# big-nacho/patolette

Measured on AMD Instinct MI355X. Metric: Mpixels/sec quantized (256-color ICtCp + KMeans) at 1 GPU; palette ΔE vs ref, higher is better.
Workload: dtype f64

## Files before the change

patolette_amd/csrc/pipeline.hip:

```cpp
#include <algorithm>
#include <functional>
#include <chrono>
#include <cmath>
#include <atomic>
#include <memory>
#include <mutex>
#include <thread>
#include <future>

#include "color_device.h"
#include "common.h"
#include "host_math.h"
#include "kmeans.h"
#include "map.h"
#include "saliency.h"
#include "quant.h"
#include "rgba.h"
#include "compact.h"

namespace pamd {

void launch_convert(int which, const double *src, double *dst, size_t n, ConvertStats *stats, hipStream_t s, BinK sumk = BinK{0.0, 0.0},
                    BinK momk = BinK{0.0, 0.0}, size_t begin = 0, size_t end = ~(size_t)0, bool init_stats = true);
void launch_convert_rows(int which, const double *rows, double *dst, size_t n, ConvertStats *stats, hipStream_t s,
// ... 818 lines not shown
    PinBuf<ConvertStats> h_cstats;
    hipEvent_t ev_stats = nullptr;
    hipStream_t stream2 = nullptr;
    hipEvent_t ev_up[2] = {nullptr, nullptr}, ev_join = nullptr;
    size_t prep_N = 0, prep_planes = 0;
    DevBuf<double> src, wsrc, cvt, bufA, bufB, aux;
    DevBuf<unsigned short> bkt;
    DevBuf<NodeDev> nodes;
    DevBuf<NodeIn> stage_in;
    DevBuf<NodeOut> stage_out;
    DevBuf<int> ids, round_nodes, node_tile0;
    DevBuf<Tile> tilesA, tilesP;
    DevBuf<double> hist, sum6, dpal;
    DevBuf<unsigned long long> hsize, tileoff;
    DevBuf<unsigned int> hcount, tilecnt;
    DevBuf<unsigned char> lut, dmap, src8, pal8, quant8;
    DevBuf<unsigned> rgba_cnt;
    DevBuf<int> rgba_cpos;
    DevBuf<unsigned char> rgba_rgb, rgba_map;
    DevBuf<double> rgba_w;
    PinBuf<unsigned> h_rgba_m;
    DevBuf<ConvertStats> cstats;
    PinBuf<NodeIn> h_stage_in;
    PinBuf<NodeOut> h_stage_out;
    PinBuf<int> h_ids, h_ids_get;
    PinBuf<Tile> h_tilesA, h_tilesP;
    PinBuf<int> h_round, h_tile0;
    PinBuf<double> h_dbl;
    PinBuf<unsigned char> h_bytes, h_packet, h_mapstage;
    DevBuf<unsigned char> packet;
// ... 402 lines not shown

static bool lq_device_eligible(const Engine &E, size_t N, size_t K, bool verbose, bool allow_device) {
    const int lq_mode = g_lq_device.load(std::memory_order_relaxed);
    return allow_device && (lq_mode == 1 || (lq_mode == 2 && N < kLqDeviceAutoPixels)) && !E.shard && !verbose && K <= (size_t)kLqDevMaxK;
}

static void ws_prepare(Engine &E, size_t N, size_t K, bool weighted, bool verbose) {
    const size_t planes = weighted ? 4 : 3;
    const bool lq_dev = lq_device_eligible(E, N, K, verbose, true);
    const size_t slack = lq_dev ? (size_t)kLqRoundCap : 0, ntA = ceil_div(N, (size_t)kTileA) + slack, ntP = ceil_div(N, (size_t)kTileP) + slack;
    const size_t tables = lq_dev ? (size_t)kLqRoundCap * kBuckets : (size_t)kBuckets;
    E.cvt.reserve(planes * N); E.cstats.reserve(1);
    E.bufA.reserve(planes * N + 64); E.bufB.reserve(planes * N + 64); E.bkt.reserve(N);
    E.tilesA.reserve(ntA); E.tilesP.reserve(ntP);
    E.tilecnt.reserve(ntP * kMaxChildren); E.tileoff.reserve(ntP * kMaxChildren);
    E.round_nodes.reserve(1); E.node_tile0.reserve(2); E.h_round.reserve(kBuckets);
    E.hist.reserve(std::max(hist_slot_doubles(), lq_dev ? (size_t)kNQ_LQ * 2 * kBuckets * kLqRoundCap : 0));
    E.hsize.reserve(tables); E.hcount.reserve(tables); E.lut.reserve(tables);
    E.nodes.reserve(std::max<size_t>(4 * K + 64, lq_dev ? (size_t)kLqNodeCap : 0));
    E.h_dbl.reserve(16 * kBuckets * 2 + 64);
    E.gq.reserve(1); E.gqout.reserve(1); E.h_gqout.reserve(1); E.h_gq.reserve(1);
    const size_t nput = kGqMaxK + 1;
    E.stage_in.reserve(nput); E.stage_out.reserve(nput); E.ids.reserve(nput); E.h_stage_in.reserve(nput); E.h_stage_out.reserve(nput);
    E.h_ids.reserve(nput); E.h_ids_get.reserve(nput);
    E.h_cent.reserve(3 * K);
    if (lq_dev) { E.lqctl.reserve(1); E.h_lqhead.reserve(1); E.h_lqrec.reserve(kLqNodeCap); E.h_lqcen.reserve(kLqNodeCap); }
}

static int lq_device_loop(Engine &E, size_t N, size_t K, bool weighted, bool inv_sums, const Bounds &bnd, const QuantBuffers &qlq, int kbase,
                          int first_base, int nnodes, std::vector<double> &centers, size_t &len, unsigned long long *max_members) {
    hipStream_t s = E.stream;
    const size_t lqs = (size_t)kNQ_LQ * 2 * kBuckets;
    const int ntA_ub = (int)ceil_div(N, (size_t)kTileA) + kLqRoundCap, ntP_ub = (int)ceil_div(N, (size_t)kTileP) + kLqRoundCap;
    E.lqctl.reserve(1); E.h_lqhead.reserve(1); E.h_lqrec.reserve(kLqNodeCap); E.h_lqcen.reserve(kLqNodeCap);
    E.hist.reserve(std::max(hist_slot_doubles(), lqs * kLqRoundCap)); E.hsize.reserve((size_t)kLqRoundCap * kBuckets);
    E.hcount.reserve((size_t)kLqRoundCap * kBuckets); E.lut.reserve((size_t)kLqRoundCap * kBuckets);
    E.tilesA.reserve(ntA_ub); E.tilesP.reserve(ntP_ub);
    E.tilecnt.reserve((size_t)ntP_ub * kMaxChildren); E.tileoff.reserve((size_t)ntP_ub * kMaxChildren);
    LqCtl *c = E.lqctl.p;
    LqHead *head = E.h_lqhead.p;
    for (int r = 0; r < kLqMaxRounds; r++) { head->round_px[r] = 0.0; head->round_nr[r] = 0.0; }
    const RoundDyn *dyn = &c->dyn;
    const int *d_round = c->round_ids, *d_tP0 = c->tP0;
    int call = 0;
    const GqOut *gq = kbase < 0 ? (const GqOut *)E.gqout.p : nullptr;
    const int kb_ub = kbase < 0 ? kGqMaxK : kbase;
    auto control = [&]() {
        const bool first = call == 0;
        {
            KTIME("k_lq_children", s, 0.0);
            if (first) hipLaunchKernelGGL(k_lq_children, (kb_ub + 3) / 4, 256, 0, s, E.nodes.p, c, call, kb_ub, first_base, nnodes, (int)K, gq);
            else hipLaunchKernelGGL(k_lq_children, 2 * kLqRoundCap / 4, 256, 0, s, E.nodes.p, c, call, 0, 0, 0, 0, (const GqOut *)nullptr);
        }
        KTIME("k_lq_select", s, 0.0);
        hipLaunchKernelGGL(k_lq_select, 1 + (first ? (kb_ub + 3) / 4 : 2 * kLqRoundCap / 4), 256, 0, s, E.nodes.p, c, call, bnd.e_lin, bnd.e_quad);
        HIP_CHECK(hipGetLastError());
        call++;
    };
    int enq = 0;
    auto round = [&]() {
        if (enq >= kLqMaxRounds) throw HipError("patolette_amd: split loop exceeded its round limit");
        const double *px_src = &head->round_px[enq], *nr_src = &head->round_nr[enq];
        const bool rev = enq % 2 == 1;
        static const bool setup_kernel = getenv("PAMD_LQ_SETUP_KERNEL") && atoi(getenv("PAMD_LQ_SETUP_KERNEL")) != 0;
        if (setup_kernel) {
            hipLaunchKernelGGL(k_round_setup_dyn, 1024, 256, 0, s, E.nodes.p, (const LqCtl *)c, E.tilesA.p, E.tilesP.p, E.hist.p, E.hsize.p, E.hcount.p, lqs);
            HIP_CHECK(hipGetLastError());
            launch_minmax(qlq, E.tilesA.p, ntA_ub, 0, E.nodes.p, s, rev, dyn, px_src);
        } else {
            const RoundLists rl{c->round_ids, c->tA0, c->tP0, E.tilesA.p, E.tilesP.p, E.hist.p, lqs, E.hsize.p, E.hcount.p};
            launch_minmax(qlq, E.tilesA.p, ntA_ub, 0, E.nodes.p, s, rev, dyn, px_src, &rl);
        }
        launch_hist(qlq, false, E.tilesA.p, ntA_ub, 0, E.nodes.p, E.hist.p, E.hsize.p, E.hcount.p, s, !rev, false, dyn, px_src);
        launch_cut(weighted, E.nodes.p, d_round, kLqRoundCap, E.hist.p, E.hsize.p, E.hcount.p, E.lut.p, s, dyn, nr_src);
        launch_partition(qlq, E.tilesP.p, ntP_ub, 0, d_round, d_tP0, kLqRoundCap, E.nodes.p, E.lut.p, E.tilecnt.p, E.tileoff.p, true, s, inv_sums, rev, dyn, px_src);
        enq++;
        control();
    };
    control();
    int want = (E.lq_hint_N == N && E.lq_hint_K == K && E.lq_hint_rounds > 0) ? E.lq_hint_rounds : 9;
    const bool fault_full = g_debug_fault.load(std::memory_order_relaxed) == 4;
    if (fault_full) want = 3;
    for (;;) {
        while (enq < want) round();
        hipLaunchKernelGGL(k_lq_export, 16, 256, 0, s, (const LqCtl *)c, head, E.h_lqrec.p, E.h_lqcen.p);
        HIP_CHECK(hipGetLastError());
        E.sync();
        if (fault_full) return -2;
        if (head->done) break;
        want = enq + 2;
// ... 1918 lines not shown
```

patolette_amd/csrc/quant.h:

```cpp
#pragma once

#include <atomic>

#include "common.h"
#include "devutil.h"

namespace pamd {

constexpr int kMaxChildren = 16;
constexpr int kTileA = 8192;
constexpr int kTileP = 2048;

constexpr int kNQ_LQ = 4;
constexpr int kNQ_GQ = 14;

constexpr int kSlots = 16;

struct NodeIn {
    unsigned long long begin, n, gn;
    int buf, slot, child0, nchild;
    int split;
    double axis[3], mean[3], sw;
    BinK klin, kquad;
};
// ... 84 lines not shown
constexpr int kSum3Slots = 32;
void launch_sum3(const double *planar, size_t N, BinK k, double *d_out6, hipStream_t s);
constexpr int kGqMaxK = 12;
struct GqDpDev {
    unsigned long long w0[kBuckets + 1];
    double w1[3][kBuckets + 1], w2[kBuckets + 1];
    double E[2][kBuckets + 1];
    int cut[kGqMaxK + 1][kBuckets + 1];
};
void launch_gq_dp(const double *d_hist, const unsigned int *d_hcount, int kmax, GqDpDev *d_g, hipStream_t s);

void launch_minmax(const QuantBuffers &qb, const Tile *d_tiles, int ntiles, size_t px, NodeDev *d_nodes, hipStream_t s, bool from_end = false,
                   const RoundDyn *dyn = nullptr, const double *px_src = nullptr, const RoundLists *lists = nullptr);
void launch_hist(const QuantBuffers &qb, bool gq, const Tile *d_tiles, int ntiles, size_t px, NodeDev *d_nodes,
                 double *d_hist, unsigned long long *d_hsize, unsigned int *d_hcount, hipStream_t s, bool from_end = false,
                 bool fixed_point = false, const RoundDyn *dyn = nullptr, const double *px_src = nullptr);
void launch_cut(bool weighted, NodeDev *d_nodes, const int *d_round_nodes, int nround, const double *d_hist,
                const unsigned long long *d_hsize, const unsigned int *d_hcount, unsigned char *d_lut, hipStream_t s,
                const RoundDyn *dyn = nullptr, const double *nr_src = nullptr);
void launch_partition(const QuantBuffers &qb, const Tile *d_ptiles, int nptiles, size_t px, const int *d_round_nodes,
                      const int *d_node_tile0, int nround, NodeDev *d_nodes, const unsigned char *d_lut,
                      unsigned int *d_tilecnt, unsigned long long *d_tileoff, bool fuse_cov, hipStream_t s,
                      bool invariant = false, bool from_end = false, const RoundDyn *dyn = nullptr, const double *px_src = nullptr,
                      bool gated = false);
void launch_cov_children(const QuantBuffers &qb, const Tile *d_tiles, int ntiles, size_t px, NodeDev *d_nodes, hipStream_t s, bool from_end = false,
                         bool gated = false);
void launch_cov_nodes(const QuantBuffers &qb, const double *planar_override, const Tile *d_tiles, int ntiles, size_t px,
                      NodeDev *d_nodes, hipStream_t s, bool from_end = false);

extern std::atomic<int> g_debug_fault;
size_t hist_slot_doubles();

}
```

patolette_amd/csrc/quant.hip:

```cpp
#include "quant.h"

#include <atomic>

#include <type_traits>

namespace pamd {

template <typename T>
__device__ __forceinline__ T block_scan_incl(T v, T *smem) {
    const int lane = threadIdx.x & 63, wid = threadIdx.x >> 6, nw = blockDim.x >> 6;
#pragma unroll
    for (int o = 1; o < 64; o <<= 1) {
        T t = __shfl_up(v, o, 64);
        if (lane >= o) v += t;
    }
    __syncthreads();
    if (lane == 63) smem[wid] = v;
    __syncthreads();
    if (wid == 0) {
        T s = lane < nw ? smem[lane] : T(0);
#pragma unroll
        for (int o = 1; o < 16; o <<= 1) {
            T t = __shfl_up(s, o, 64);
            if (lane >= o) s += t;
// ... 107 lines not shown
#pragma unroll
    for (int o = 32; o > 0; o >>= 1) { mn = fmin(mn, __shfl_down(mn, o, 64)); mx = fmax(mx, __shfl_down(mx, o, 64)); }
    __shared__ double smn[4], smx[4];
    if ((threadIdx.x & 63) == 0) { smn[threadIdx.x >> 6] = mn; smx[threadIdx.x >> 6] = mx; }
    __syncthreads();
    if (threadIdx.x == 0) {
        for (int w = 1; w < 4; w++) { mn = fmin(mn, smn[w]); mx = fmax(mx, smx[w]); }
        if (mn <= mx) {
            atomicMin(&nd.minkey[blockIdx.x & (kSlots - 1)], f64_key(mn));
            atomicMax(&nd.maxkey[blockIdx.x & (kSlots - 1)], f64_key(mx));
        }
    }
}

constexpr int kHistCombineMin = 12;
template <bool W, bool GQ>
__global__ __launch_bounds__(512) void k_hist(QuantBuffers qb, const Tile *__restrict__ tiles, int ntiles, NodeDev *nodes,
                                              double *hist, unsigned long long *hsize, unsigned int *hcount, const int from_end,
                                              const RoundDyn *__restrict__ dyn) {
    constexpr int NQ = GQ ? (W ? 14 : 10) : (W ? 4 : 3);
    int nblk = (int)gridDim.x;
    if (dyn) {
        ntiles = dyn->ntA;
        nblk = min(ntiles, nblk);
        if ((int)blockIdx.x >= nblk) return;
    }
    constexpr int NQS = GQ ? kNQ_GQ : kNQ_LQ;
    extern __shared__ double lds[];
    double *h = lds;
    unsigned long long *siz = (unsigned long long *)(h + NQ * 2 * kBuckets);
    unsigned int *cnt = (unsigned int *)(siz + kBuckets);
    for (int i = threadIdx.x; i < NQ * 2 * kBuckets; i += blockDim.x) h[i] = 0.0;
    for (int i = threadIdx.x; i < kBuckets; i += blockDim.x) { cnt[i] = 0u; siz[i] = 0ULL; }
    __syncthreads();

    const int per = (ntiles + nblk - 1) / nblk;
    const int bid = from_end ? nblk - 1 - (int)blockIdx.x : (int)blockIdx.x;
    const int tfirst = bid * per, tlast = min(ntiles, tfirst + per);
    for (int ti = tfirst; ti < tlast; ti++) {
        const Tile t = tiles[ti];
        NodeDev &nd = nodes[t.node];
        const double a0 = nd.axis[0], a1 = nd.axis[1], a2 = nd.axis[2];
        double mn, mx;
        node_minmax(nd, mn, mx);
        const bool degenerate = (mx - mn < kDelta);
        const double sc = 1 / (mx - mn);
        const BinK klin = nd.klin, kquad = nd.kquad;
        const double *px = qb.buf[nd.buf], *py = px + qb.N, *pz = py + qb.N, *pw = pz + qb.N;
// ... 62 lines not shown
        for (; i + 512 < t.count; i += 1024) {
            const size_t p0 = t.start + i, p1 = p0 + 512;
            const double x0 = px[p0], y0 = py[p0], z0 = pz[p0], x1 = px[p1], y1 = py[p1], z1 = pz[p1];
            double w0 = 1.0, w1 = 1.0;
            if constexpr (W) { w0 = pw[p0]; w1 = pw[p1]; }
            one(p0, x0, y0, z0, w0);
            one(p1, x1, y1, z1, w1);
        }
        for (; i < t.count; i += 512) {
            const size_t p = t.start + i;
            double w = 1.0;
            if constexpr (W) w = pw[p];
            one(p, px[p], py[p], pz[p], w);
        }
        const bool flush = (ti + 1 == tlast) || tiles[ti + 1].node != t.node;
        if (!flush) continue;
        __syncthreads();
        const size_t slot = (size_t)nd.slot;
        double *gh = hist + slot * (size_t)(NQS * 2 * kBuckets);
        for (int i = threadIdx.x; i < NQ * 2 * kBuckets; i += blockDim.x) {
            double v = h[i];
            if (v != 0.0) { unsafeAtomicAdd(&gh[i], v); h[i] = 0.0; }
        }
        for (int b = threadIdx.x; b < kBuckets; b += blockDim.x) {
            unsigned c = cnt[b];
            if (c) { atomicAdd(&hcount[slot * kBuckets + b], c); cnt[b] = 0u; }
            if constexpr (W && !GQ) { const unsigned long long s = siz[b]; if (s) { atomicAdd(&hsize[slot * kBuckets + b], s); siz[b] = 0ULL; } }
        }
        __syncthreads();
    }
}

// ... 133 lines not shown
                h[i2] = 0ULL;
            }
        }
        for (int b = threadIdx.x; b < kBuckets; b += blockDim.x) {
            unsigned c = cnt[b];
            if (c) { atomicAdd(&hcount[slot * kBuckets + b], c); cnt[b] = 0u; }
            if constexpr (W && !GQ) { const unsigned long long s2 = siz[b]; if (s2) { atomicAdd(&hsize[slot * kBuckets + b], s2); siz[b] = 0ULL; } }
        }
        __syncthreads();
    }
}

template <bool W>
__global__ __launch_bounds__(512) void k_cut(NodeDev *nodes, const int *__restrict__ round_nodes, const double *__restrict__ hist,
                                             const unsigned long long *__restrict__ hsize, const unsigned int *__restrict__ hcount,
                                             unsigned char *lut, const int fault, const RoundDyn *__restrict__ dyn) {
    if (dyn && (int)blockIdx.x >= dyn->nr) return;
    __shared__ double sd[4 * 16];
    __shared__ unsigned long long su[2 * 16];
    __shared__ double best_v[8];
    __shared__ int best_i[8];
    __shared__ double tot[8];
    __shared__ unsigned long long tots[2];
    __shared__ int s_split;
    const int b = threadIdx.x;
    NodeDev &nd = nodes[round_nodes[blockIdx.x]];
    const size_t slot = (size_t)nd.slot;
    const double *gh = hist + slot * (size_t)(kNQ_LQ * 2 * kBuckets);
    constexpr int NQ = W ? 4 : 3;
    double p[NQ][2];
    {
// ... 67 lines not shown
            double s0[NQ], s1[NQ];
#pragma unroll
            for (int q = 0; q < NQ; q++) {
                s0[q] = side == 0 ? p[q][0] : tot[q * 2] - p[q][0];
                s1[q] = side == 0 ? p[q][1] : tot[q * 2 + 1] - p[q][1];
            }
            double sw = W ? (s0[NQ - 1] + s1[NQ - 1]) : (double)ch.n;
            ch.sw = sw;
            const double inv = 1 / sw;
            for (int j = 0; j < 3; j++) ch.mean[j] = (s0[j] + s1[j]) * inv;
            ch.axis[0] = ch.axis[1] = ch.axis[2] = 0;
        }
    }
    for (int i = b; i < 2 * kNodeResetElems; i += kBuckets)
        node_reset_element(nodes[nd.child0 + i / kNodeResetElems], i % kNodeResetElems);
}

__global__ __launch_bounds__(256) void k_count(QuantBuffers qb, const Tile *__restrict__ tiles, const NodeDev *__restrict__ nodes,
                                               const unsigned char *__restrict__ lut, unsigned int *tilecnt, const int from_end,
                                               const RoundDyn *__restrict__ dyn) {
    __shared__ unsigned int c[kMaxChildren];
    __shared__ unsigned char sl[kBuckets];
    const unsigned nt = dyn ? (unsigned)dyn->ntP : gridDim.x;
    if (blockIdx.x >= nt) return;
    const unsigned tix = from_end ? nt - 1u - blockIdx.x : blockIdx.x;
    const Tile t = tiles[tix];
    const NodeDev &nd = nodes[t.node];
    const unsigned char *l = lut + (size_t)nd.slot * kBuckets;
    if (threadIdx.x < kMaxChildren) c[threadIdx.x] = 0;
    const int nch = nd.nchild;
// ... 162 lines not shown
            const int ch = (int)(cr[r] & 255u);
            if (ch != 255) {
                const size_t src = t.start + r * 256 + threadIdx.x;
                const size_t dst = off[r][wid][ch] + (cr[r] >> 8);
                const double x = sx[src], y = sy[src], z = sz[src];
                double w = 1.0;
                if constexpr (W) w = sw[src];
                dx[dst] = x; dy[dst] = y; dz[dst] = z;
                if constexpr (W) dw[dst] = w;
            }
        }
        __syncthreads();
    }
}

template <bool W, bool INV>
__global__ __launch_bounds__(256, (W || INV) ? 2 : 3) void k_scatter_bin(QuantBuffers qb, const Tile *__restrict__ tiles, int ntiles, NodeDev *nodes,
                                                                        const NodeDev *__restrict__ nodes_ro,
                                                                        const unsigned long long *__restrict__ tileoff, const int from_end,
                                                                        const RoundDyn *__restrict__ dyn) {
    constexpr int R = kTileP / 256;
    static_assert(R * 4 == 32, "one 32-lane group per child");
    __shared__ unsigned int wcnt[2][2][R * 4];
    __shared__ double sm[28 * 4];
    const int lane = threadIdx.x & 63, wid = __builtin_amdgcn_readfirstlane((int)(threadIdx.x >> 6));
    const unsigned long long ltmask = (1ULL << lane) - 1ULL;
    int nblk = (int)gridDim.x;
    if ((from_end & 2) && nodes_ro[0].nchild != 2) return;
    if (dyn) {
        ntiles = dyn->ntP;
        nblk = min(ntiles, nblk);
        if ((int)blockIdx.x >= nblk) return;
    }
    const int per = (ntiles + nblk - 1) / nblk;
    const int bid = (from_end & 1) ? nblk - 1 - (int)blockIdx.x : (int)blockIdx.x;
    const int tfirst = bid * per, tlast = min(ntiles, tfirst + per);
    if (tfirst >= tlast) return;
    constexpr int NP = INV ? 14 : 7;
    double pl[NP], pr[NP];
#pragma unroll
    for (int i = 0; i < NP; i++) { pl[i] = 0; pr[i] = 0; }

    auto fetch_buckets = [&](const Tile &tt, const int ti, unsigned (&b)[R], unsigned long long &toff) {
        const unsigned last = tt.count - 1u;
#pragma unroll
        for (int r = 0; r < R; r++) b[r] = qb.bkt[tt.start + min((unsigned)(r * 256) + threadIdx.x, last)];
        toff = tileoff[(size_t)ti * kMaxChildren + (lane >> 5)];
    };
    auto classify = [&](const Tile &tt, const unsigned (&b)[R], const int split, const int par, unsigned (&cr)[R]) {
#pragma unroll
        for (int r = 0; r < R; r++) {
            const bool valid = (unsigned)(r * 256) + threadIdx.x < tt.count;
            const bool right = (int)b[r] > split;
            const unsigned long long mR = __ballot(valid && right), mL = __ballot(valid && !right);
            const unsigned rk = (unsigned)__popcll((right ? mR : mL) & ltmask);
            cr[r] = (valid ? (right ? 1u : 0u) : 2u) | (rk << 8);
            if (lane == 0) { wcnt[par][0][r * 4 + wid] = (unsigned)__popcll(mL); wcnt[par][1][r * 4 + wid] = (unsigned)__popcll(mR); }
        }
    };
    auto lane64 = [](const unsigned long long v, const int l) {
        return ((unsigned long long)(unsigned)__builtin_amdgcn_readlane((int)(unsigned)(v >> 32), l) << 32) |
               (unsigned)__builtin_amdgcn_readlane((int)(unsigned)v, l);
    };
    Tile t = tiles[tfirst];
    unsigned cr[R];
    unsigned long long baseL, baseR;
    {
        unsigned b0[R];
        unsigned long long toff;
        fetch_buckets(t, tfirst, b0, toff);
        classify(t, b0, nodes_ro[t.node].split, 0, cr);
        baseL = lane64(toff, 0); baseR = lane64(toff, 32);
    }
    for (int ti = tfirst; ti < tlast; ti++) {
        const int par = (ti - tfirst) & 1;
        const NodeDev &nd = nodes_ro[t.node];
        const int child0 = nd.child0;
        const double *sx = qb.buf[nd.buf], *sy = sx + qb.N, *sz = sy + qb.N, *sw = sz + qb.N;
        double *dx = qb.buf[1 - nd.buf], *dy = dx + qb.N, *dz = dy + qb.N, *dw = dz + qb.N;
        double x[R], y[R], z[R], w[R];
        {
            const unsigned last = t.count - 1u;
#pragma unroll
            for (int r = 0; r < R; r++) {
                const size_t src = t.start + min((unsigned)(r * 256) + threadIdx.x, last);
                x[r] = sx[src]; y[r] = sy[src]; z[r] = sz[src];
                w[r] = 1.0;
                if constexpr (W) w[r] = sw[src];
            }
        }
        const bool more = ti + 1 < tlast;
        const int tnx = more ? ti + 1 : ti;
        const Tile tn = tiles[tnx];
        unsigned bkn[R];
        unsigned long long toffn;
        fetch_buckets(tn, tnx, bkn, toffn);
        __syncthreads();
        const unsigned c = wcnt[par][lane >> 5][lane & 31];
        const unsigned incl = wave_scan_incl_u32(c);
        const unsigned tot0 = (unsigned)__builtin_amdgcn_readlane((int)incl, 31);
        const unsigned excl = incl - c - (lane >= 32 ? tot0 : 0u);
        const NodeDev &c0 = nodes_ro[child0], &c1 = nodes_ro[child0 + 1];
        const double m0L = c0.mean[0], m1L = c0.mean[1], m2L = c0.mean[2], m0R = c1.mean[0], m1R = c1.mean[1], m2R = c1.mean[2];
        BinK kinv{0.0, 0.0};
        if constexpr (INV) kinv = nd.kquad;
        const size_t slack = (size_t)(W ? 4 : 3) * qb.N + (size_t)lane;
#pragma unroll
        for (int r = 0; r < R; r++) {
            const unsigned eL = (unsigned)__builtin_amdgcn_readlane((int)excl, r * 4 + wid);
            const unsigned eR = (unsigned)__builtin_amdgcn_readlane((int)excl, 32 + r * 4 + wid);
            const unsigned ch = cr[r] & 255u;
// ... 34 lines not shown
                }
            }
            block_sum<28>(a, sm);
            if (threadIdx.x == 0) {
                for (int side = 0; side < 2; side++) {
                    NodeDev &chn = nodes[child0 + side];
                    for (int i = 0; i < 7; i++) {
                        if (a[14 * side + 2 * i] != 0.0) unsafeAtomicAdd(&chn.acc[blockIdx.x & (kSlots - 1)][i][0], a[14 * side + 2 * i]);
                        if (a[14 * side + 2 * i + 1] != 0.0) unsafeAtomicAdd(&chn.acc[blockIdx.x & (kSlots - 1)][i][1], a[14 * side + 2 * i + 1]);
                    }
                }
            }
        }
        if (more) {
            classify(tn, bkn, nodes_ro[tn.node].split, par ^ 1, cr);
            baseL = lane64(toffn, 0); baseR = lane64(toffn, 32);
        }
        t = tn;
    }
}

template <bool W>
__device__ __forceinline__ void cov_accumulate(const double *px, const double *py, const double *pz, const double *pw,
                                               size_t lo, size_t hi, const double m0, const double m1, const double m2,
                                               const BinK kq, double (&a)[14]) {
    for (size_t p = lo + threadIdx.x; p < hi; p += blockDim.x) {
        double dx = px[p] - m0, dy = py[p] - m1, dz = pz[p] - m2;
        double w = 1.0;
        if constexpr (W) w = pw[p];
        double wx = w * dx, wy = w * dy, wz = w * dz;
        bin_add(wx * dx, kq, a[0], a[1]);
// ... 70 lines not shown
static void launch_hist_fix(const QuantBuffers &qb, const Tile *d_tiles, int ntiles, size_t px, NodeDev *d_nodes, double *d_hist,
                            unsigned long long *d_hsize, unsigned int *d_hcount, hipStream_t s, bool from_end) {
    constexpr int NQ = W ? 14 : 10;
    const size_t lds = (size_t)NQ * kBuckets * sizeof(unsigned long long) + kBuckets * (sizeof(unsigned int) + sizeof(unsigned long long));
    static PerDeviceOnce attr_set;
    attr_set.once([&] { HIP_CHECK(hipFuncSetAttribute((const void *)k_hist_fix<W, true>, hipFuncAttributeMaxDynamicSharedMemorySize, (int)lds)); });
    KTIME("k_hist_gq", s, (W ? 34.0 : 26.0) * px);
    const int g = std::min(ntiles, 256 * (W ? 2 : 3));
    hipLaunchKernelGGL((k_hist_fix<W, true>), g, 512, lds, s, qb, d_tiles, ntiles, d_nodes, d_hist, d_hsize, d_hcount, from_end ? 1 : 0);
    HIP_CHECK(hipGetLastError());
}

template <bool W, bool GQ>
static void launch_hist_t(const QuantBuffers &qb, const Tile *d_tiles, int ntiles, size_t px, NodeDev *d_nodes, double *d_hist,
                          unsigned long long *d_hsize, unsigned int *d_hcount, hipStream_t s, bool from_end,
                          const RoundDyn *dyn = nullptr, const double *px_src = nullptr) {
    constexpr int NQ = GQ ? (W ? 14 : 10) : (W ? 4 : 3);
    size_t lds = (size_t)NQ * 2 * kBuckets * sizeof(double) + kBuckets * (sizeof(unsigned int) + sizeof(unsigned long long));
    static PerDeviceOnce attr_set;
    attr_set.once([&] { HIP_CHECK(hipFuncSetAttribute((const void *)k_hist<W, GQ>, hipFuncAttributeMaxDynamicSharedMemorySize, (int)lds)); });
    KTIME_DYN(GQ ? "k_hist_gq" : "k_hist_lq", s, (W ? 34.0 : 26.0), px, px_src);
    const int g = std::min(ntiles, 256 * (GQ ? 1 : 4));
    hipLaunchKernelGGL((k_hist<W, GQ>), g, 512, lds, s, qb, d_tiles, ntiles, d_nodes, d_hist, d_hsize, d_hcount, from_end ? 1 : 0, dyn);
    HIP_CHECK(hipGetLastError());
}

__global__ __launch_bounds__(512) void k_gq_prefix(const double *__restrict__ hist, const unsigned int *__restrict__ hcount, GqDpDev *g) {
    __shared__ double sh[4][kBuckets + 1];
    __shared__ unsigned long long sc[kBuckets + 1];
    const int b = threadIdx.x;
#pragma unroll
    for (int hq = 0; hq < 4; hq++)
        sh[hq][b + 1] = hist[(size_t)(hq * 2 + 0) * kBuckets + b] + hist[(size_t)(hq * 2 + 1) * kBuckets + b];
    sc[b + 1] = hcount[b];
    if (b < 4) sh[b][0] = 0;
    if (b == 4) sc[0] = 0;
    __syncthreads();
    if (b == 0) { unsigned long long a = 0; for (int i = 1; i <= kBuckets; i++) { a += sc[i]; sc[i] = a; } }
// ... 45 lines not shown
        En[n] = e;
        g->cut[k][n] = cut;
    }
}

void launch_gq_dp(const double *d_hist, const unsigned int *d_hcount, int kmax, GqDpDev *d_g, hipStream_t s) {
    KTIME("k_gq_dp", s, (double)kmax * 513 * 513 * 8);
    hipLaunchKernelGGL(k_gq_prefix, 1, 512, 0, s, d_hist, d_hcount, d_g);
    hipLaunchKernelGGL(k_gq_init, 3, 256, 0, s, d_g);
    for (int k = 2; k <= kmax; k++) hipLaunchKernelGGL(k_gq_dp, kBuckets + 1, 256, 0, s, d_g, k);
    HIP_CHECK(hipGetLastError());
}

void launch_hist(const QuantBuffers &qb, bool gq, const Tile *d_tiles, int ntiles, size_t px, NodeDev *d_nodes,
                 double *d_hist, unsigned long long *d_hsize, unsigned int *d_hcount, hipStream_t s, bool from_end, bool fixed_point,
                 const RoundDyn *dyn, const double *px_src) {
    if (!ntiles) return;
    if (gq && fixed_point) {
        if (qb.weighted) launch_hist_fix<true>(qb, d_tiles, ntiles, px, d_nodes, d_hist, d_hsize, d_hcount, s, from_end);
        else launch_hist_fix<false>(qb, d_tiles, ntiles, px, d_nodes, d_hist, d_hsize, d_hcount, s, from_end);
        return;
    }
    if (qb.weighted) { if (gq) launch_hist_t<true, true>(qb, d_tiles, ntiles, px, d_nodes, d_hist, d_hsize, d_hcount, s, from_end);
                       else launch_hist_t<true, false>(qb, d_tiles, ntiles, px, d_nodes, d_hist, d_hsize, d_hcount, s, from_end, dyn, px_src); }
    else { if (gq) launch_hist_t<false, true>(qb, d_tiles, ntiles, px, d_nodes, d_hist, d_hsize, d_hcount, s, from_end);
           else launch_hist_t<false, false>(qb, d_tiles, ntiles, px, d_nodes, d_hist, d_hsize, d_hcount, s, from_end, dyn, px_src); }
}

std::atomic<int> g_debug_fault{0};
void launch_cut(bool weighted, NodeDev *d_nodes, const int *d_round_nodes, int nround, const double *d_hist,
                const unsigned long long *d_hsize, const unsigned int *d_hcount, unsigned char *d_lut, hipStream_t s, const RoundDyn *dyn, const double *nr_src) {
    if (!nround) return;
    KTIME_DYN("k_cut", s, (double)kNQ_LQ * 2 * kBuckets * 8, nround, nr_src);
    const int fault = g_debug_fault.load(std::memory_order_relaxed);
    if (weighted) hipLaunchKernelGGL(k_cut<true>, nround, 512, 0, s, d_nodes, d_round_nodes, d_hist, d_hsize, d_hcount, d_lut, fault, dyn);
    else hipLaunchKernelGGL(k_cut<false>, nround, 512, 0, s, d_nodes, d_round_nodes, d_hist, d_hsize, d_hcount, d_lut, fault, dyn);
    HIP_CHECK(hipGetLastError());
}

void launch_partition(const QuantBuffers &qb, const Tile *d_ptiles, int nptiles, size_t px, const int *d_round_nodes,
                      const int *d_node_tile0, int nround, NodeDev *d_nodes, const unsigned char *d_lut,
                      unsigned int *d_tilecnt, unsigned long long *d_tileoff, bool fuse_cov, hipStream_t s, bool invariant, bool from_end,
                      const RoundDyn *dyn, const double *px_src, bool gated) {
    const int fe = (from_end ? 1 : 0) | (gated ? 2 : 0);
    if (!nround) return;
    if (nptiles) { KTIME_DYN("k_count", s, 2.0, px, px_src); hipLaunchKernelGGL(k_count, nptiles, 256, 0, s, qb, d_ptiles, d_nodes, d_lut, d_tilecnt, fe & 1, dyn); }
    { KTIME_DYN("k_scan", s, 12.0 * kMaxChildren / (double)kTileP, dyn ? px : (size_t)nptiles * kTileP, px_src);
      hipLaunchKernelGGL(k_scan, nround, 1024, 0, s, d_round_nodes, d_node_tile0, d_nodes, d_tilecnt, d_tileoff, dyn); }
    if (nptiles) {
        KTIME_DYN(fuse_cov ? "k_scatter_cov" : "k_scatter", s, (qb.weighted ? 66.0 : 50.0), px, px_src);
        if (fuse_cov) {
            const int gb = std::min(nptiles, 256 * ((invariant || qb.weighted) ? 2 : 3));
            if (invariant) {
                if (qb.weighted) hipLaunchKernelGGL((k_scatter_bin<true, true>), gb, 256, 0, s, qb, d_ptiles, nptiles, d_nodes, (const NodeDev *)d_nodes, d_tileoff, fe, dyn);
                else hipLaunchKernelGGL((k_scatter_bin<false, true>), gb, 256, 0, s, qb, d_ptiles, nptiles, d_nodes, (const NodeDev *)d_nodes, d_tileoff, fe, dyn);
            } else if (qb.weighted) hipLaunchKernelGGL((k_scatter_bin<true, false>), gb, 256, 0, s, qb, d_ptiles, nptiles, d_nodes, (const NodeDev *)d_nodes, d_tileoff, fe, dyn);
            else hipLaunchKernelGGL((k_scatter_bin<false, false>), gb, 256, 0, s, qb, d_ptiles, nptiles, d_nodes, (const NodeDev *)d_nodes, d_tileoff, fe, dyn);
            if (gated) {
                HIP_CHECK(hipGetLastError());
                const int fg = (from_end ? 1 : 0) | 4;
                if (qb.weighted) hipLaunchKernelGGL((k_scatter<true>), nptiles, 256, 0, s, qb, d_ptiles, nptiles, d_nodes, d_lut, d_tileoff, fg);
                else hipLaunchKernelGGL((k_scatter<false>), nptiles, 256, 0, s, qb, d_ptiles, nptiles, d_nodes, d_lut, d_tileoff, fg);
            }
        } else {
            if (qb.weighted) hipLaunchKernelGGL((k_scatter<true>), nptiles, 256, 0, s, qb, d_ptiles, nptiles, d_nodes, d_lut, d_tileoff, fe);
            else hipLaunchKernelGGL((k_scatter<false>), nptiles, 256, 0, s, qb, d_ptiles, nptiles, d_nodes, d_lut, d_tileoff, fe);
        }
    }
    HIP_CHECK(hipGetLastError());
}

void launch_cov_children(const QuantBuffers &qb, const Tile *d_tiles, int ntiles, size_t px, NodeDev *d_nodes, hipStream_t s, bool from_end, bool gated) {
    if (!ntiles) return;
    KTIME("k_cov", s, (qb.weighted ? 32.0 : 24.0) * px);
    const int fe = (from_end ? 1 : 0) | (gated ? 4 : 0);
    if (qb.weighted) hipLaunchKernelGGL(k_cov_children<true>, ntiles, 256, 0, s, qb, d_tiles, d_nodes, fe);
    else hipLaunchKernelGGL(k_cov_children<false>, ntiles, 256, 0, s, qb, d_tiles, d_nodes, fe);
    HIP_CHECK(hipGetLastError());
}

void launch_cov_nodes(const QuantBuffers &qb, const double *planar_override, const Tile *d_tiles, int ntiles, size_t px,
                      NodeDev *d_nodes, hipStream_t s, bool from_end) {
    if (!ntiles) return;
// ... 8 lines not shown
```

Measured before the change: 3134.

## Derive partition offsets from per-tile histogram CDFs instead of separate count/scan

In the device-side split loop, the histogram kernel now writes a per-streaming-tile cumulative bucket count (tcdf). The cut kernel reads the CDF at the chosen split to compute per-tile left/right output offsets directly. A new scatter variant then uses these offsets, recomputing sub-tile prefixes from bucket data, which removes the k_count and k_scan launches and the tilecnt/tileoff passes from each round. The cost is extra per-tile syncs and scans plus 16-bit CDF stores in k_hist, and a launch-bounds change that alters occupancy.

```diff
diff --git a/patolette_amd/csrc/pipeline.hip b/patolette_amd/csrc/pipeline.hip
--- a/patolette_amd/csrc/pipeline.hip
+++ b/patolette_amd/csrc/pipeline.hip
@@ -856,6 +856,8 @@
     DevBuf<double> hist, sum6, dpal;
     DevBuf<unsigned long long> hsize, tileoff;
     DevBuf<unsigned int> hcount, tilecnt;
+    DevBuf<unsigned short> tcdf;
+    DevBuf<ulonglong2> toffA;
     DevBuf<unsigned char> lut, dmap, src8, pal8, quant8;
     DevBuf<unsigned> rgba_cnt;
     DevBuf<int> rgba_cpos;
@@ -1288,6 +1290,7 @@
     E.bufA.reserve(planes * N + 64); E.bufB.reserve(planes * N + 64); E.bkt.reserve(N);
     E.tilesA.reserve(ntA); E.tilesP.reserve(ntP);
     E.tilecnt.reserve(ntP * kMaxChildren); E.tileoff.reserve(ntP * kMaxChildren);
+    if (lq_dev) { E.tcdf.reserve(ntA * kBuckets); E.toffA.reserve(ntA); }
     E.round_nodes.reserve(1); E.node_tile0.reserve(2); E.h_round.reserve(kBuckets);
     E.hist.reserve(std::max(hist_slot_doubles(), lq_dev ? (size_t)kNQ_LQ * 2 * kBuckets * kLqRoundCap : 0));
     E.hsize.reserve(tables); E.hcount.reserve(tables); E.lut.reserve(tables);
@@ -1310,12 +1313,12 @@
     E.hist.reserve(std::max(hist_slot_doubles(), lqs * kLqRoundCap)); E.hsize.reserve((size_t)kLqRoundCap * kBuckets);
     E.hcount.reserve((size_t)kLqRoundCap * kBuckets); E.lut.reserve((size_t)kLqRoundCap * kBuckets);
     E.tilesA.reserve(ntA_ub); E.tilesP.reserve(ntP_ub);
-    E.tilecnt.reserve((size_t)ntP_ub * kMaxChildren); E.tileoff.reserve((size_t)ntP_ub * kMaxChildren);
+    E.tcdf.reserve((size_t)ntA_ub * kBuckets); E.toffA.reserve(ntA_ub);
     LqCtl *c = E.lqctl.p;
     LqHead *head = E.h_lqhead.p;
     for (int r = 0; r < kLqMaxRounds; r++) { head->round_px[r] = 0.0; head->round_nr[r] = 0.0; }
     const RoundDyn *dyn = &c->dyn;
-    const int *d_round = c->round_ids, *d_tP0 = c->tP0;
+    const int *d_round = c->round_ids;
     int call = 0;
     const GqOut *gq = kbase < 0 ? (const GqOut *)E.gqout.p : nullptr;
     const int kb_ub = kbase < 0 ? kGqMaxK : kbase;
@@ -1345,9 +1348,9 @@
             const RoundLists rl{c->round_ids, c->tA0, c->tP0, E.tilesA.p, E.tilesP.p, E.hist.p, lqs, E.hsize.p, E.hcount.p};
             launch_minmax(qlq, E.tilesA.p, ntA_ub, 0, E.nodes.p, s, rev, dyn, px_src, &rl);
         }
-        launch_hist(qlq, false, E.tilesA.p, ntA_ub, 0, E.nodes.p, E.hist.p, E.hsize.p, E.hcount.p, s, !rev, false, dyn, px_src);
-        launch_cut(weighted, E.nodes.p, d_round, kLqRoundCap, E.hist.p, E.hsize.p, E.hcount.p, E.lut.p, s, dyn, nr_src);
-        launch_partition(qlq, E.tilesP.p, ntP_ub, 0, d_round, d_tP0, kLqRoundCap, E.nodes.p, E.lut.p, E.tilecnt.p, E.tileoff.p, true, s, inv_sums, rev, dyn, px_src);
+        launch_hist(qlq, false, E.tilesA.p, ntA_ub, 0, E.nodes.p, E.hist.p, E.hsize.p, E.hcount.p, s, !rev, false, dyn, px_src, E.tcdf.p);
+        launch_cut(weighted, E.nodes.p, d_round, kLqRoundCap, E.hist.p, E.hsize.p, E.hcount.p, E.lut.p, s, dyn, nr_src, c->tA0, E.tcdf.p, E.toffA.p);
+        launch_partition_bin_ta(qlq, E.tilesP.p, ntP_ub, 0, E.nodes.p, E.toffA.p, c->tA0, s, inv_sums, rev, dyn, px_src);
         enq++;
         control();
     };
diff --git a/patolette_amd/csrc/quant.h b/patolette_amd/csrc/quant.h
--- a/patolette_amd/csrc/quant.h
+++ b/patolette_amd/csrc/quant.h
@@ -122,15 +122,18 @@
                    const RoundDyn *dyn = nullptr, const double *px_src = nullptr, const RoundLists *lists = nullptr);
 void launch_hist(const QuantBuffers &qb, bool gq, const Tile *d_tiles, int ntiles, size_t px, NodeDev *d_nodes,
                  double *d_hist, unsigned long long *d_hsize, unsigned int *d_hcount, hipStream_t s, bool from_end = false,
-                 bool fixed_point = false, const RoundDyn *dyn = nullptr, const double *px_src = nullptr);
+                 bool fixed_point = false, const RoundDyn *dyn = nullptr, const double *px_src = nullptr, unsigned short *d_tcdf = nullptr);
 void launch_cut(bool weighted, NodeDev *d_nodes, const int *d_round_nodes, int nround, const double *d_hist,
                 const unsigned long long *d_hsize, const unsigned int *d_hcount, unsigned char *d_lut, hipStream_t s,
-                const RoundDyn *dyn = nullptr, const double *nr_src = nullptr);
+                const RoundDyn *dyn = nullptr, const double *nr_src = nullptr, const int *d_tA0 = nullptr,
+                const unsigned short *d_tcdf = nullptr, ulonglong2 *d_toffA = nullptr);
 void launch_partition(const QuantBuffers &qb, const Tile *d_ptiles, int nptiles, size_t px, const int *d_round_nodes,
                       const int *d_node_tile0, int nround, NodeDev *d_nodes, const unsigned char *d_lut,
                       unsigned int *d_tilecnt, unsigned long long *d_tileoff, bool fuse_cov, hipStream_t s,
                       bool invariant = false, bool from_end = false, const RoundDyn *dyn = nullptr, const double *px_src = nullptr,
                       bool gated = false);
+void launch_partition_bin_ta(const QuantBuffers &qb, const Tile *d_ptiles, int nptiles, size_t px, NodeDev *d_nodes, const ulonglong2 *d_toffA,
+                             const int *d_tA0, hipStream_t s, bool invariant, bool from_end, const RoundDyn *dyn, const double *px_src);
 void launch_cov_children(const QuantBuffers &qb, const Tile *d_tiles, int ntiles, size_t px, NodeDev *d_nodes, hipStream_t s, bool from_end = false,
                          bool gated = false);
 void launch_cov_nodes(const QuantBuffers &qb, const double *planar_override, const Tile *d_tiles, int ntiles, size_t px,
diff --git a/patolette_amd/csrc/quant.hip b/patolette_amd/csrc/quant.hip
--- a/patolette_amd/csrc/quant.hip
+++ b/patolette_amd/csrc/quant.hip
@@ -145,11 +145,12 @@
 }
 
 constexpr int kHistCombineMin = 12;
-template <bool W, bool GQ>
-__global__ __launch_bounds__(512) void k_hist(QuantBuffers qb, const Tile *__restrict__ tiles, int ntiles, NodeDev *nodes,
+template <bool W, bool GQ, bool CDF>
+__global__ __launch_bounds__(512, (CDF && !W) ? 8 : 1) void k_hist(QuantBuffers qb, const Tile *__restrict__ tiles, int ntiles, NodeDev *nodes,
                                               double *hist, unsigned long long *hsize, unsigned int *hcount, const int from_end,
-                                              const RoundDyn *__restrict__ dyn) {
+                                              const RoundDyn *__restrict__ dyn, unsigned short *tcdf) {
     constexpr int NQ = GQ ? (W ? 14 : 10) : (W ? 4 : 3);
+    static_assert(kBuckets == 512, "one bucket per thread of the block (tcdf)");
     int nblk = (int)gridDim.x;
     if (dyn) {
         ntiles = dyn->ntA;
@@ -163,6 +164,8 @@
     unsigned int *cnt = (unsigned int *)(siz + kBuckets);
     for (int i = threadIdx.x; i < NQ * 2 * kBuckets; i += blockDim.x) h[i] = 0.0;
     for (int i = threadIdx.x; i < kBuckets; i += blockDim.x) { cnt[i] = 0u; siz[i] = 0ULL; }
+    [[maybe_unused]] __shared__ unsigned int wtot[8];
+    [[maybe_unused]] unsigned int cnt_prev = 0u;
     __syncthreads();
 
     const int per = (ntiles + nblk - 1) / nblk;
@@ -255,8 +258,25 @@
             one(p, px[p], py[p], pz[p], w);
         }
         const bool flush = (ti + 1 == tlast) || tiles[ti + 1].node != t.node;
-        if (!flush) continue;
-        __syncthreads();
+        if constexpr (CDF) {
+            {
+                __syncthreads();
+                const unsigned c = cnt[threadIdx.x];
+                unsigned v = c - cnt_prev;
+                cnt_prev = flush ? 0u : c;
+                v = wave_scan_incl_u32(v);
+                if ((threadIdx.x & 63) == 63) wtot[threadIdx.x >> 6] = v;
+                __syncthreads();
+                const int wid = (int)(threadIdx.x >> 6);
+#pragma unroll
+                for (int w = 0; w < 7; w++) v += w < wid ? wtot[w] : 0u;
+                tcdf[(size_t)ti * kBuckets + threadIdx.x] = (unsigned short)v;
+                if (!flush) continue;
+            }
+        } else {
+            if (!flush) continue;
+            __syncthreads();
+        }
         const size_t slot = (size_t)nd.slot;
         double *gh = hist + slot * (size_t)(NQS * 2 * kBuckets);
         for (int i = threadIdx.x; i < NQ * 2 * kBuckets; i += blockDim.x) {
@@ -420,7 +440,8 @@
 template <bool W>
 __global__ __launch_bounds__(512) void k_cut(NodeDev *nodes, const int *__restrict__ round_nodes, const double *__restrict__ hist,
                                              const unsigned long long *__restrict__ hsize, const unsigned int *__restrict__ hcount,
-                                             unsigned char *lut, const int fault, const RoundDyn *__restrict__ dyn) {
+                                             unsigned char *lut, const int fault, const RoundDyn *__restrict__ dyn,
+                                             const int *__restrict__ tA0, const unsigned short *__restrict__ tcdf, ulonglong2 *toffA) {
     if (dyn && (int)blockIdx.x >= dyn->nr) return;
     __shared__ double sd[4 * 16];
     __shared__ unsigned long long su[2 * 16];
@@ -518,6 +539,38 @@
     }
     for (int i = b; i < 2 * kNodeResetElems; i += kBuckets)
         node_reset_element(nodes[nd.child0 + i / kNodeResetElems], i % kNodeResetElems);
+    if (!tcdf) return;
+    const int t0 = tA0[blockIdx.x], t1 = tA0[blockIdx.x + 1];
+    const int C = (t1 - t0 + kBuckets - 1) / kBuckets;
+    const int ga = min(t1, t0 + b * C), gb = min(t1, ga + C);
+    const unsigned long long n = nd.n, base = nd.begin;
+    auto tile_px = [&](const int g) {
+        const unsigned long long o = (unsigned long long)(g - t0) * kTileA;
+        return (unsigned)(n - o < (unsigned long long)kTileA ? n - o : (unsigned long long)kTileA);
+    };
+    unsigned long long sum[2] = {0, 0};
+    for (int g = ga; g < gb; g += 8) {
+        unsigned v[8];
+#pragma unroll
+        for (int q = 0; q < 8; q++) v[q] = g + q < gb ? (unsigned)tcdf[(size_t)(g + q) * kBuckets + split] : 0u;
+#pragma unroll
+        for (int q = 0; q < 8; q++) if (g + q < gb) { sum[0] += v[q]; sum[1] += tile_px(g + q) - v[q]; }
+    }
+    unsigned long long inc[2] = {sum[0], sum[1]};
+    block_scan_incl_vec<unsigned long long, 2>(inc, su);
+    __shared__ unsigned long long s_left;
+    if (b == kBuckets - 1) s_left = inc[0];
+    __syncthreads();
+    const unsigned long long base1 = base + s_left;
+    unsigned long long run0 = base + inc[0] - sum[0], run1 = base1 + inc[1] - sum[1];
+    for (int g = ga; g < gb; g += 8) {
+        unsigned v[8];
+#pragma unroll
+        for (int q = 0; q < 8; q++) v[q] = g + q < gb ? (unsigned)tcdf[(size_t)(g + q) * kBuckets + split] : 0u;
+#pragma unroll
+        for (int q = 0; q < 8; q++)
+            if (g + q < gb) { toffA[g + q] = make_ulonglong2(run0, run1); run0 += v[q]; run1 += tile_px(g + q) - v[q]; }
+    }
 }
 
 __global__ __launch_bounds__(256) void k_count(QuantBuffers qb, const Tile *__restrict__ tiles, const NodeDev *__restrict__ nodes,
@@ -710,12 +763,14 @@
     }
 }
 
-template <bool W, bool INV>
+template <bool W, bool INV, bool TA>
 __global__ __launch_bounds__(256, (W || INV) ? 2 : 3) void k_scatter_bin(QuantBuffers qb, const Tile *__restrict__ tiles, int ntiles, NodeDev *nodes,
                                                                         const NodeDev *__restrict__ nodes_ro,
                                                                         const unsigned long long *__restrict__ tileoff, const int from_end,
-                                                                        const RoundDyn *__restrict__ dyn) {
+                                                                        const RoundDyn *__restrict__ dyn, const int *__restrict__ tA0) {
     constexpr int R = kTileP / 256;
+    constexpr int kSub = kTileA / kTileP;
+    static_assert(kTileA % kTileP == 0, "a streaming tile is a whole number of partition tiles");
     static_assert(R * 4 == 32, "one 32-lane group per child");
     __shared__ unsigned int wcnt[2][2][R * 4];
     __shared__ double sm[28 * 4];
@@ -741,7 +796,7 @@
         const unsigned last = tt.count - 1u;
 #pragma unroll
         for (int r = 0; r < R; r++) b[r] = qb.bkt[tt.start + min((unsigned)(r * 256) + threadIdx.x, last)];
-        toff = tileoff[(size_t)ti * kMaxChildren + (lane >> 5)];
+        toff = tileoff[(size_t)ti * (TA ? 2 : kMaxChildren) + (lane >> 5)];
     };
     auto classify = [&](const Tile &tt, const unsigned (&b)[R], const int split, const int par, unsigned (&cr)[R]) {
 #pragma unroll
@@ -761,12 +816,36 @@
     Tile t = tiles[tfirst];
     unsigned cr[R];
     unsigned long long baseL, baseR;
+    [[maybe_unused]] int ai = 0, q = 0;
+    if constexpr (TA) {
+        const NodeDev &n0 = nodes_ro[t.node];
+        const int j = (int)((t.start - n0.begin) / (unsigned long long)kTileP);
+        ai = tA0[n0.slot] + j / kSub; q = j % kSub;
+    }
     {
         unsigned b0[R];
         unsigned long long toff;
-        fetch_buckets(t, tfirst, b0, toff);
-        classify(t, b0, nodes_ro[t.node].split, 0, cr);
+        const int split = nodes_ro[t.node].split;
+        fetch_buckets(t, TA ? ai : tfirst, b0, toff);
+        classify(t, b0, split, 0, cr);
         baseL = lane64(toff, 0); baseR = lane64(toff, 32);
+        if constexpr (TA) {
+            if (q > 0) {
+                typedef unsigned short us8 __attribute__((ext_vector_type(8), aligned(2)));
+                __shared__ unsigned int wleft[4];
+                unsigned left = 0;
+                for (int s = q; s > 0; s--) {
+                    const us8 v = *reinterpret_cast<const us8 *>(qb.bkt + (t.start - (size_t)s * kTileP) + threadIdx.x * 8u);
+#pragma unroll
+                    for (int e = 0; e < 8; e++) left += (int)v[e] > split ? 0u : 1u;
+                }
+                left = wave_sum_u32(left);
+                if (lane == 0) wleft[wid] = left;
+                __syncthreads();
+                const unsigned before = (unsigned)__builtin_amdgcn_readfirstlane((int)(wleft[0] + wleft[1] + wleft[2] + wleft[3]));
+                baseL += before; baseR += (unsigned)q * (unsigned)kTileP - before;
+            }
+        }
     }
     for (int ti = tfirst; ti < tlast; ti++) {
         const int par = (ti - tfirst) & 1;
@@ -788,9 +867,11 @@
         const bool more = ti + 1 < tlast;
         const int tnx = more ? ti + 1 : ti;
         const Tile tn = tiles[tnx];
+        const bool same_ta = TA && more && q + 1 < kSub && tn.node == t.node;
+        const int ain = (same_ta || !more) ? ai : ai + 1;
         unsigned bkn[R];
         unsigned long long toffn;
-        fetch_buckets(tn, tnx, bkn, toffn);
+        fetch_buckets(tn, TA ? ain : tnx, bkn, toffn);
         __syncthreads();
         const unsigned c = wcnt[par][lane >> 5][lane & 31];
         const unsigned incl = wave_scan_incl_u32(c);
@@ -855,7 +936,8 @@
         }
         if (more) {
             classify(tn, bkn, nodes_ro[tn.node].split, par ^ 1, cr);
-            baseL = lane64(toffn, 0); baseR = lane64(toffn, 32);
+            if (same_ta) { baseL += tot0; baseR += t.count - tot0; q++; }
+            else { baseL = lane64(toffn, 0); baseR = lane64(toffn, 32); q = 0; ai = ain; }
         }
         t = tn;
     }
@@ -956,14 +1038,24 @@
 template <bool W, bool GQ>
 static void launch_hist_t(const QuantBuffers &qb, const Tile *d_tiles, int ntiles, size_t px, NodeDev *d_nodes, double *d_hist,
                           unsigned long long *d_hsize, unsigned int *d_hcount, hipStream_t s, bool from_end,
-                          const RoundDyn *dyn = nullptr, const double *px_src = nullptr) {
+                          const RoundDyn *dyn = nullptr, const double *px_src = nullptr, unsigned short *d_tcdf = nullptr) {
     constexpr int NQ = GQ ? (W ? 14 : 10) : (W ? 4 : 3);
     size_t lds = (size_t)NQ * 2 * kBuckets * sizeof(double) + kBuckets * (sizeof(unsigned int) + sizeof(unsigned long long));
     static PerDeviceOnce attr_set;
-    attr_set.once([&] { HIP_CHECK(hipFuncSetAttribute((const void *)k_hist<W, GQ>, hipFuncAttributeMaxDynamicSharedMemorySize, (int)lds)); });
+    attr_set.once([&] {
+        HIP_CHECK(hipFuncSetAttribute((const void *)k_hist<W, GQ, false>, hipFuncAttributeMaxDynamicSharedMemorySize, (int)lds));
+        if constexpr (!GQ) HIP_CHECK(hipFuncSetAttribute((const void *)k_hist<W, GQ, true>, hipFuncAttributeMaxDynamicSharedMemorySize, (int)lds));
+    });
     KTIME_DYN(GQ ? "k_hist_gq" : "k_hist_lq", s, (W ? 34.0 : 26.0), px, px_src);
     const int g = std::min(ntiles, 256 * (GQ ? 1 : 4));
-    hipLaunchKernelGGL((k_hist<W, GQ>), g, 512, lds, s, qb, d_tiles, ntiles, d_nodes, d_hist, d_hsize, d_hcount, from_end ? 1 : 0, dyn);
+    if constexpr (!GQ) {
+        if (d_tcdf) {
+            hipLaunchKernelGGL((k_hist<W, GQ, true>), g, 512, lds, s, qb, d_tiles, ntiles, d_nodes, d_hist, d_hsize, d_hcount, from_end ? 1 : 0, dyn, d_tcdf);
+            HIP_CHECK(hipGetLastError());
+            return;
+        }
+    }
+    hipLaunchKernelGGL((k_hist<W, GQ, false>), g, 512, lds, s, qb, d_tiles, ntiles, d_nodes, d_hist, d_hsize, d_hcount, from_end ? 1 : 0, dyn, nullptr);
     HIP_CHECK(hipGetLastError());
 }
 
@@ -1039,7 +1131,7 @@
 
 void launch_hist(const QuantBuffers &qb, bool gq, const Tile *d_tiles, int ntiles, size_t px, NodeDev *d_nodes,
                  double *d_hist, unsigned long long *d_hsize, unsigned int *d_hcount, hipStream_t s, bool from_end, bool fixed_point,
-                 const RoundDyn *dyn, const double *px_src) {
+                 const RoundDyn *dyn, const double *px_src, unsigned short *d_tcdf) {
     if (!ntiles) return;
     if (gq && fixed_point) {
         if (qb.weighted) launch_hist_fix<true>(qb, d_tiles, ntiles, px, d_nodes, d_hist, d_hsize, d_hcount, s, from_end);
@@ -1047,19 +1139,20 @@
         return;
     }
     if (qb.weighted) { if (gq) launch_hist_t<true, true>(qb, d_tiles, ntiles, px, d_nodes, d_hist, d_hsize, d_hcount, s, from_end);
-                       else launch_hist_t<true, false>(qb, d_tiles, ntiles, px, d_nodes, d_hist, d_hsize, d_hcount, s, from_end, dyn, px_src); }
+                       else launch_hist_t<true, false>(qb, d_tiles, ntiles, px, d_nodes, d_hist, d_hsize, d_hcount, s, from_end, dyn, px_src, d_tcdf); }
     else { if (gq) launch_hist_t<false, true>(qb, d_tiles, ntiles, px, d_nodes, d_hist, d_hsize, d_hcount, s, from_end);
-           else launch_hist_t<false, false>(qb, d_tiles, ntiles, px, d_nodes, d_hist, d_hsize, d_hcount, s, from_end, dyn, px_src); }
+           else launch_hist_t<false, false>(qb, d_tiles, ntiles, px, d_nodes, d_hist, d_hsize, d_hcount, s, from_end, dyn, px_src, d_tcdf); }
 }
 
 std::atomic<int> g_debug_fault{0};
 void launch_cut(bool weighted, NodeDev *d_nodes, const int *d_round_nodes, int nround, const double *d_hist,
-                const unsigned long long *d_hsize, const unsigned int *d_hcount, unsigned char *d_lut, hipStream_t s, const RoundDyn *dyn, const double *nr_src) {
+                const unsigned long long *d_hsize, const unsigned int *d_hcount, unsigned char *d_lut, hipStream_t s, const RoundDyn *dyn, const double *nr_src,
+                const int *d_tA0, const unsigned short *d_tcdf, ulonglong2 *d_toffA) {
     if (!nround) return;
     KTIME_DYN("k_cut", s, (double)kNQ_LQ * 2 * kBuckets * 8, nround, nr_src);
     const int fault = g_debug_fault.load(std::memory_order_relaxed);
-    if (weighted) hipLaunchKernelGGL(k_cut<true>, nround, 512, 0, s, d_nodes, d_round_nodes, d_hist, d_hsize, d_hcount, d_lut, fault, dyn);
-    else hipLaunchKernelGGL(k_cut<false>, nround, 512, 0, s, d_nodes, d_round_nodes, d_hist, d_hsize, d_hcount, d_lut, fault, dyn);
+    if (weighted) hipLaunchKernelGGL(k_cut<true>, nround, 512, 0, s, d_nodes, d_round_nodes, d_hist, d_hsize, d_hcount, d_lut, fault, dyn, d_tA0, d_tcdf, d_toffA);
+    else hipLaunchKernelGGL(k_cut<false>, nround, 512, 0, s, d_nodes, d_round_nodes, d_hist, d_hsize, d_hcount, d_lut, fault, dyn, d_tA0, d_tcdf, d_toffA);
     HIP_CHECK(hipGetLastError());
 }
 
@@ -1077,10 +1170,10 @@
         if (fuse_cov) {
             const int gb = std::min(nptiles, 256 * ((invariant || qb.weighted) ? 2 : 3));
             if (invariant) {
-                if (qb.weighted) hipLaunchKernelGGL((k_scatter_bin<true, true>), gb, 256, 0, s, qb, d_ptiles, nptiles, d_nodes, (const NodeDev *)d_nodes, d_tileoff, fe, dyn);
-                else hipLaunchKernelGGL((k_scatter_bin<false, true>), gb, 256, 0, s, qb, d_ptiles, nptiles, d_nodes, (const NodeDev *)d_nodes, d_tileoff, fe, dyn);
-            } else if (qb.weighted) hipLaunchKernelGGL((k_scatter_bin<true, false>), gb, 256, 0, s, qb, d_ptiles, nptiles, d_nodes, (const NodeDev *)d_nodes, d_tileoff, fe, dyn);
-            else hipLaunchKernelGGL((k_scatter_bin<false, false>), gb, 256, 0, s, qb, d_ptiles, nptiles, d_nodes, (const NodeDev *)d_nodes, d_tileoff, fe, dyn);
+                if (qb.weighted) hipLaunchKernelGGL((k_scatter_bin<true, true, false>), gb, 256, 0, s, qb, d_ptiles, nptiles, d_nodes, (const NodeDev *)d_nodes, d_tileoff, fe, dyn, nullptr);
+                else hipLaunchKernelGGL((k_scatter_bin<false, true, false>), gb, 256, 0, s, qb, d_ptiles, nptiles, d_nodes, (const NodeDev *)d_nodes, d_tileoff, fe, dyn, nullptr);
+            } else if (qb.weighted) hipLaunchKernelGGL((k_scatter_bin<true, false, false>), gb, 256, 0, s, qb, d_ptiles, nptiles, d_nodes, (const NodeDev *)d_nodes, d_tileoff, fe, dyn, nullptr);
+            else hipLaunchKernelGGL((k_scatter_bin<false, false, false>), gb, 256, 0, s, qb, d_ptiles, nptiles, d_nodes, (const NodeDev *)d_nodes, d_tileoff, fe, dyn, nullptr);
             if (gated) {
                 HIP_CHECK(hipGetLastError());
                 const int fg = (from_end ? 1 : 0) | 4;
@@ -1092,6 +1185,21 @@
             else hipLaunchKernelGGL((k_scatter<false>), nptiles, 256, 0, s, qb, d_ptiles, nptiles, d_nodes, d_lut, d_tileoff, fe);
         }
     }
+    HIP_CHECK(hipGetLastError());
+}
+
+void launch_partition_bin_ta(const QuantBuffers &qb, const Tile *d_ptiles, int nptiles, size_t px, NodeDev *d_nodes, const ulonglong2 *d_toffA,
+                             const int *d_tA0, hipStream_t s, bool invariant, bool from_end, const RoundDyn *dyn, const double *px_src) {
+    if (!nptiles) return;
+    KTIME_DYN("k_scatter_cov", s, (qb.weighted ? 66.0 : 50.0), px, px_src);
+    const int gb = std::min(nptiles, 256 * ((invariant || qb.weighted) ? 2 : 3));
+    const int fe = from_end ? 1 : 0;
+    const unsigned long long *off = (const unsigned long long *)d_toffA;
+    if (invariant) {
+        if (qb.weighted) hipLaunchKernelGGL((k_scatter_bin<true, true, true>), gb, 256, 0, s, qb, d_ptiles, nptiles, d_nodes, (const NodeDev *)d_nodes, off, fe, dyn, d_tA0);
+        else hipLaunchKernelGGL((k_scatter_bin<false, true, true>), gb, 256, 0, s, qb, d_ptiles, nptiles, d_nodes, (const NodeDev *)d_nodes, off, fe, dyn, d_tA0);
+    } else if (qb.weighted) hipLaunchKernelGGL((k_scatter_bin<true, false, true>), gb, 256, 0, s, qb, d_ptiles, nptiles, d_nodes, (const NodeDev *)d_nodes, off, fe, dyn, d_tA0);
+    else hipLaunchKernelGGL((k_scatter_bin<false, false, true>), gb, 256, 0, s, qb, d_ptiles, nptiles, d_nodes, (const NodeDev *)d_nodes, off, fe, dyn, d_tA0);
     HIP_CHECK(hipGetLastError());
 }
 
```

Result: faster. 3213, median of 6 (+2.5%).
